# louissmit/VBNN

Hardware: AMD Instinct MI355X
Metric: VBLinear fwd+bwd samples/sec (higher is better)
Workload: dtype bf16; 1 GPU; 784-4096-4096-10 VBLinear MLP, batch 4096 per GPU, LRT, S=1; mode=lrt, global_batch=4096, parallelism=dp1, warmup_steps_run=255, backward_order=every updateGradInput, then the accGradParameters from the first layer up, launch=one stream launch per kernel

## Files before the change

include/vbnn_hip.h:

```cpp
#ifndef VBNN_HIP_H
#define VBNN_HIP_H

#include <stddef.h>
#include <stdint.h>

#ifdef __cplusplus
extern "C" {
#endif
#if defined(__GNUC__)
#pragma GCC visibility push(default)
#endif

#define VBNN_ABI_VERSION 6
#define VBNN_KPAD 64

enum { VBNN_OK = 0, VBNN_ERR_INVALID = 1, VBNN_ERR_HIP = 2, VBNN_ERR_NOMEM = 3, VBNN_ERR_UNSUPPORTED = 4 };
enum { VBNN_F32 = 0, VBNN_BF16 = 1 };
enum { VBNN_PACK_COPY = 0, VBNN_PACK_EXP = 1, VBNN_PACK_SQUARE = 2, VBNN_PACK_MUL = 3,
       VBNN_PACK_RELU = 4, VBNN_PACK_RELU_SQUARE = 5 };

typedef struct vbnn_ctx vbnn_ctx;

int vbnn_abi_version(void);
const char* vbnn_last_error(void);

#define VBNN_DEBUG_GEMM_KERNEL 0
#define VBNN_DEBUG_V2_SCHEDULE 1
#define VBNN_DEBUG_V2_TILE 2
#define VBNN_DEBUG_V3_MIN_K 4
#define VBNN_DEBUG_V2_PSPLIT 5
#define VBNN_DEBUG_V3_SPLIT 8
#define VBNN_DEBUG_V0 9
#define VBNN_DEBUG_HEAD_BACKWARD 10
#define VBNN_DEBUG_KMAJOR 6
int vbnn_debug_set(int key, int value);
#define VBNN_DEBUG_LAST_HEAD_FORM 11
#define VBNN_HEAD_ENTRY_FORWARD 1
#define VBNN_HEAD_ENTRY_SLOTS 2
#define VBNN_HEAD_ENTRY_STEP 3
#define VBNN_HEAD_ENTRY_TILE 4
#define VBNN_HEAD_ENTRY_STREAM 5
#define VBNN_HEAD_FINISH_NONE 0
#define VBNN_HEAD_FINISH_INLINE 1
#define VBNN_HEAD_FINISH_KERNEL 2
#define VBNN_HEAD_FORM(entry, bf16, vec, full, cp, finish) ((entry) | ((bf16) << 4) | ((vec) << 5) | ((full) << 6) | ((cp) << 8) | ((finish) << 16))
int vbnn_debug_get(int key);

int vbnn_kmajor_supported(int64_t M, int64_t N, int64_t K);
int vbnn_kmajor_supported_dw(int64_t I, int64_t O, int64_t N, int bias_row);
int vbnn_ctx_kmajor_supported(vbnn_ctx* ctx, int64_t M, int64_t N, int64_t K);
int vbnn_ctx_kmajor_supported_dw(vbnn_ctx* ctx, int64_t I, int64_t O, int64_t N, int bias_row);

int vbnn_ctx_create(int device, void* hip_stream, vbnn_ctx** out);
int vbnn_ctx_create_cu_budget(int device, int n_cus, vbnn_ctx** out);
int vbnn_ctx_stream(vbnn_ctx* ctx, void** hip_stream_out, int* n_cus_out);
int vbnn_ctx_destroy(vbnn_ctx* ctx);
int vbnn_ctx_set_stream(vbnn_ctx* ctx, void* hip_stream);
int vbnn_sync(vbnn_ctx* ctx);

int vbnn_buf_alloc(vbnn_ctx* ctx, size_t bytes, void** dptr);
int vbnn_buf_free(vbnn_ctx* ctx, void* dptr);
int vbnn_buf_zero(vbnn_ctx* ctx, void* dptr, size_t bytes);
int vbnn_buf_upload(vbnn_ctx* ctx, void* dst_dev, const void* src_host, size_t bytes);
int vbnn_buf_download(vbnn_ctx* ctx, void* dst_host, const void* src_dev, size_t bytes);

int vbnn_fill_normal(vbnn_ctx* ctx, float* out, int64_t rows, int64_t cols, int64_t ld,
                     uint64_t seed, uint32_t stream, uint32_t layer, uint32_t draw, int64_t row0,
                     float scale);
int vbnn_fill_normal_hw(vbnn_ctx* ctx, float* out, int64_t rows, int64_t cols, int64_t ld,
                        uint64_t seed, uint32_t stream, uint32_t layer, uint32_t draw, int64_t row0,
                        float scale);

int vbnn_box_muller_forms(vbnn_ctx* ctx, const uint32_t* x0, const uint32_t* x1, float* z_exact, float* z_hw, int64_t n);

int vbnn_compute_prior(vbnn_ctx* ctx, const float* means, const float* lvars, int64_t W,
                       float* vars, float* stdv, float* mu_sqe, double* stats);

int vbnn_wn_sample(vbnn_ctx* ctx, const float* means, const float* stdv, const float* lvars,
                   float* weight, float* e_out, int64_t O, int64_t I,
                   uint64_t seed, uint32_t layer, uint32_t draw);

int vbnn_pack(vbnn_ctx* ctx, int dtype, int func, const float* src, const float* src2, int64_t ld_src,
              int64_t rows, int64_t cols, void* dst, int64_t ld_dst, void* dstT, int64_t ld_dstT);


typedef struct vbnn_fwd_args {
    const void* w;
    const void* w2;
    const void* x;
    const void* x2;
    int64_t ld_w, ld_x;
    int64_t N, I, O;
    const float* bias;
    uint64_t seed; uint32_t layer; uint32_t draw; int64_t row0;
    float* y;  int64_t ld_y;
    void* r;  int64_t ld_r;
    int r_packed;
    int relu;
    void* h;  void* h2;  int64_t ld_h;
    void* hT; void* h2T; int64_t ld_hT;
    int64_t rows_per_draw;
    const uint32_t* draw_dev;
    const void* head_w3; int64_t head_ld_w; int64_t head_C; float* head_slots;
} vbnn_fwd_args;

int vbnn_forward(vbnn_ctx* ctx, int dtype, const vbnn_fwd_args* a);
int vbnn_forward_head_slots(vbnn_ctx* ctx, int dtype, int64_t N, int64_t I, int64_t O, int64_t C);

typedef struct vbnn_dx_args {
    const void* wT;
    const void* w2T;
    const void* g;
    const void* gv;
    int64_t ld_wT, ld_g;
    int64_t N, I, O;
    const void* x; int64_t ld_x;
    float* gx; int64_t ld_gx;
// ... 380 lines not shown
```

vbnn_amd/csrc/epilogues.h:

```cpp
#pragma once
#include "common.h"

template <typename T> struct V4;
template <> struct V4<float> { typedef f32x4 type; };
template <> struct V4<bf16_t> { typedef bf16x4 type; };
template <typename T>
__device__ __forceinline__ void store4_out(T* base, unsigned off, float a, float b, float c, float d) {
    vbnn_store_out(base, off, typename V4<T>::type{Elt<T>::to(a), Elt<T>::to(b), Elt<T>::to(c), Elt<T>::to(d)});
}

template <typename T>
struct EpiFwd {
    typedef T elem_t;
    const float* bias;
    int noise;
    uint64_t seed; uint32_t layer, draw; int64_t row0;
    const uint32_t* draw_dev = nullptr;
    int rpd;
    float* y; int64_t ld_y; int y_vec;
    float* r; T* r_t; int64_t ld_r; int r_vec;
    int relu;
    T* h; T* h2; int64_t ld_h;
    T* hT; T* h2T; int64_t ld_hT;
    int O, N;
// ... 64 lines not shown
            }
            if (STORE_T && hT) {
#pragma unroll
                for (int j = 0; j < 4; ++j)
                    if (j < valid) {
                        hT[(int64_t)(m + j) * ld_hT + n] = Elt<T>::to(t1[j]);
                        if (h2T) h2T[(int64_t)(m + j) * ld_hT + n] = Elt<T>::to(t2[j]);
                    }
            }
        }
    }
    __device__ __forceinline__ void operator()(int m, int n, f32x4 a1, f32x4 a2) const {
        float t1[4], t2[4];
        apply<true>(m, n, a1, a2, t1, t2);
    }

    static constexpr int FAST_BATCH = 8;
    static constexpr int FAST_BATCH_V2 = 4;
    struct Pre { f32x4 b; };
    struct Lane { int nl, ml; unsigned oh, orr; };
    __host__ __device__ __forceinline__ bool fast_ok() const {
        return !y && !r && h && (ld_h % 4 == 0) && (!r_t || (r_vec && ld_r % 8 == 0 && (((uintptr_t)r_t & 15u) == 0))) &&
               (!bias || (((uintptr_t)bias & 15u) == 0)) && (int64_t)N * ld_h < (1ll << 31) && (int64_t)N * ld_r < (1ll << 31);
    }
    __device__ __forceinline__ Lane lane_init(int nl, int ml) const {
        return Lane{nl, ml, (unsigned)(nl * (int)ld_h + ml), (unsigned)(nl * (int)ld_r + ml)};
    }
    __device__ __forceinline__ Pre load_fast(int um, int un, const Lane& ln) const {
        (void)un;
        Pre p;
        p.b = bias ? *reinterpret_cast<const f32x4*>(bias + um + ln.ml) : f32x4{0.f, 0.f, 0.f, 0.f};
        return p;
    }
    struct Noise { vbnn_f32x4 z; };
    __device__ __forceinline__ Noise draw_fast(int um, int un, const Lane& ln) const {
        Noise q = {};
        if (noise) q.z = zeta4(un + ln.nl, (uint32_t)((um + ln.ml) >> 2));
        return q;
    }
    __device__ __forceinline__ void apply_fast(int um, int un, const Lane& ln, f32x4 a1, f32x4 a2, const Pre& pre, float (&t1)[4],
                                               float (&t2)[4]) const {
        apply_fast_z(um, un, ln, a1, a2, pre, draw_fast(um, un, ln), t1, t2);
    }
    __device__ __forceinline__ void apply_fast_z(int um, int un, const Lane& ln, f32x4 a1, f32x4 a2, const Pre& pre, const Noise& q,
                                                 float (&t1)[4], float (&t2)[4]) const {
        float yv[4], rv[4];
        const vbnn_f32x4 z = q.z;
#pragma unroll
        for (int j = 0; j < 4; ++j) {
            const float mb = a1[j] + pre.b[j];
            if (noise) {
                const bool pos = a2[j] > 0.f;
                const float rs = __builtin_amdgcn_rsqf(a2[j]);
                const float sd = pos ? a2[j] * rs : 0.f;
                yv[j] = fmaf(sd, z.v[j], mb);
                rv[j] = pos ? 0.5f * z.v[j] * rs : 0.f;
            } else {
                yv[j] = mb;
                rv[j] = 0.f;
            }
        }
        if (r_t) store4_out<T>(r_t + ((int64_t)un * ld_r + um), ln.orr, rv[0], rv[1], rv[2], rv[3]);
#pragma unroll
        for (int j = 0; j < 4; ++j) {
            t1[j] = relu ? fmaxf(yv[j], 0.f) : yv[j];
            const float hr = Elt<T>::from(Elt<T>::to(t1[j]));
            t2[j] = hr * hr;
        }
        const int64_t ub = (int64_t)un * ld_h + um;
        store4_out<T>(h + ub, ln.oh, t1[0], t1[1], t1[2], t1[3]);
        if (h2) store4_out<T>(h2 + ub, ln.oh, t2[0], t2[1], t2[2], t2[3]);
    }

    static constexpr int FOLD_BATCH = 1;
    static constexpr int FOLD_SERIAL = 1;
    static constexpr int FOLD_STAGE = 1;
    typedef T fold_st_t;
    __host__ __device__ __forceinline__ T* fold_st_ptr() const { return r_t; }
    __host__ __device__ __forceinline__ int64_t fold_st_ld() const { return ld_r; }
    __host__ __device__ __forceinline__ const float* fold_bias_ptr() const { return bias; }
    __device__ __forceinline__ bool fold_st_stream() const { return h2 != nullptr; }
    __device__ __forceinline__ f32x4 fold_s(int um, int un, const Lane& ln, f32x4 v, const f32x4& b4, float (&rv)[4]) const {
        const vbnn_f32x4 z = normal4(seed, layer, draw, (uint32_t)(row0 + un + ln.nl), (uint32_t)((um + ln.ml) >> 2));
        f32x4 out;
#pragma unroll
        for (int j = 0; j < 4; ++j) {
            const bool pos = v[j] > 0.f;
            const float rs = __builtin_amdgcn_rsqf(v[j]);
            const float sd = pos ? v[j] * rs : 0.f;
            out[j] = fmaf(sd, z.v[j], b4[j]);
            rv[j] = pos ? 0.5f * z.v[j] * rs : 0.f;
        }
        return out;
    }
    struct FPre { f32x4 b; };
    __device__ __forceinline__ FPre fold_load(int um, int un, const Lane& ln) const {
        (void)un;
        FPre p;
        p.b = bias ? *reinterpret_cast<const f32x4*>(bias + um + ln.ml) : f32x4{0.f, 0.f, 0.f, 0.f};
        return p;
    }
    __device__ __forceinline__ f32x4 fold(int um, int un, const Lane& ln, f32x4 v, const FPre& fp) const {
        const vbnn_f32x4 z = normal4(seed, layer, draw, (uint32_t)(row0 + un + ln.nl), (uint32_t)((um + ln.ml) >> 2));
        f32x4 out;
        float rv[4];
#pragma unroll
        for (int j = 0; j < 4; ++j) {
            const bool pos = v[j] > 0.f;
            const float rs = __builtin_amdgcn_rsqf(v[j]);
            const float sd = pos ? v[j] * rs : 0.f;
            out[j] = fmaf(sd, z.v[j], fp.b[j]);
            rv[j] = pos ? 0.5f * z.v[j] * rs : 0.f;
        }
        if (r_t) store4_out<T>(r_t + ((int64_t)un * ld_r + um), ln.orr, rv[0], rv[1], rv[2], rv[3]);
        return out;
    }
    __device__ __forceinline__ bool folded_pre_needed() const { return false; }
    __device__ __forceinline__ Pre load_folded(int, int, const Lane&) const { return Pre{f32x4{0.f, 0.f, 0.f, 0.f}}; }
    __device__ __forceinline__ void apply_folded(int um, int un, const Lane& ln, f32x4 a, f32x4, const Pre&, float (&t1)[4],
                                                 float (&t2)[4]) const {
#pragma unroll
        for (int j = 0; j < 4; ++j) {
            t1[j] = relu ? fmaxf(a[j], 0.f) : a[j];
            const float hr = Elt<T>::from(Elt<T>::to(t1[j]));
            t2[j] = hr * hr;
        }
        const int64_t ub = (int64_t)un * ld_h + um;
        store4_out<T>(h + ub, ln.oh, t1[0], t1[1], t1[2], t1[3]);
        if (h2) store4_out<T>(h2 + ub, ln.oh, t2[0], t2[1], t2[2], t2[3]);
    }
};

template <typename T>
struct EpiDx {
    typedef T elem_t;
    int dual;
    const T* x; int64_t ld_x;
    float* gx; int64_t ld_gx; int gx_vec;
    int relu_mask;
    const float* r_prev; const T* r_prev_t; int64_t ld_r_prev; int r_vec;
    T* g_prev; T* gv_prev; int64_t ld_gp;
    T* gT_prev; T* gvT_prev; int64_t ld_gpT;
    int I, N;

    static constexpr bool SPLITTABLE = false;
    static constexpr bool EDGE_FAST = false;
    static constexpr bool HEAD = false;
    __device__ __forceinline__ void bind_draw() {}
    __host__ __device__ __forceinline__ bool has_draw_dev() const { return false; }
    __device__ __forceinline__ void edge_row(int, float) const {}
    __device__ __forceinline__ void set_part(int) {}
    __host__ __device__ __forceinline__ T* t1_ptr() const { return gT_prev; }
    __host__ __device__ __forceinline__ T* t2_ptr() const { return gvT_prev; }
    __host__ __device__ __forceinline__ int64_t t_ld() const { return ld_gpT; }
    __device__ __forceinline__ int m_dim() const { return I; }
    __device__ __forceinline__ int n_dim() const { return N; }
    __host__ __device__ __forceinline__ bool v3_ok() const { return true; }

    template <bool STORE_T>
    __device__ __forceinline__ void apply(int m, int n, f32x4 a1, f32x4 a2, float (&t1)[4], float (&t2)[4]) const {
        const int valid = min(4, I - m);
#pragma unroll
        for (int j = 0; j < 4; ++j) { t1[j] = 0.f; t2[j] = 0.f; }
        if (valid <= 0 || n >= N) return;
        float xv[4] = {0.f, 0.f, 0.f, 0.f};
        if (x) load4<T>(x + (int64_t)n * ld_x + m, xv, valid, (ld_x & 3) == 0);
// ... 316 lines not shown
```

vbnn_amd/csrc/gemm.hip:

```cpp
#include "gemm_dispatch.h"

extern "C" int vbnn_debug_set(int key, int value) {
    if (key == VBNN_DEBUG_GEMM_KERNEL && value >= 0 && value <= 3) { g_force_kernel = value; return VBNN_OK; }
    if (key == VBNN_DEBUG_V2_SCHEDULE && (value == -1 || value == 0 || value == 2 || value == 4)) { g_v2_sched = value; return VBNN_OK; }
    if (key == VBNN_DEBUG_V2_TILE && (value == 0 || value == 64 || value == 128 || value == 256)) { g_v2_tile = value; return VBNN_OK; }
    if (key == VBNN_DEBUG_V3_MIN_K && value >= 64) { g_v3_min_k = value; return VBNN_OK; }
    if (key == VBNN_DEBUG_V2_PSPLIT && value >= -1 && value <= 1) { g_v2_psplit = value; return VBNN_OK; }
    if (key == VBNN_DEBUG_KMAJOR && value >= 0 && value <= 2) { g_kmajor = value; return VBNN_OK; }
    if (key == VBNN_DEBUG_V3_SPLIT && value >= -1 && value <= 1) { g_v3_split = value; return VBNN_OK; }
    if (key == VBNN_DEBUG_V0 && (value == 0 || value == 1)) { g_v0 = value; return VBNN_OK; }
    if (key == VBNN_DEBUG_HEAD_BACKWARD && value >= -1 && value <= 1) { g_head_stream = value; return VBNN_OK; }
    vbnn_set_error("vbnn_debug_set: unknown key %d / value %d", key, value);
    return VBNN_ERR_INVALID;
}
extern "C" int vbnn_debug_get(int key) { return key == VBNN_DEBUG_LAST_HEAD_FORM ? g_last_head_form : -1; }

extern "C" int vbnn_kmajor_supported(int64_t M, int64_t N, int64_t K) { return kmajor_selected(M, N, K) ? 1 : 0; }
extern "C" int vbnn_ctx_kmajor_supported(vbnn_ctx* ctx, int64_t M, int64_t N, int64_t K) {
    vbnn_cu_scope plan(ctx);
    return kmajor_selected(M, N, K) ? 1 : 0;
}
extern "C" int vbnn_kmajor_supported_dw(int64_t I, int64_t O, int64_t N, int bias_row) {
    if (!bias_row && kmajor_selected(I, O, N)) return 1;
    if (I % 4 == 0 && kmajor_dw_v3_split_selected(I + (bias_row ? 1 : 0), O, N)) return 2;
    return kmajor_dw_v2_selected(I + (bias_row ? 1 : 0), O, N) ? 1 : 0;
}
extern "C" int vbnn_ctx_kmajor_supported_dw(vbnn_ctx* ctx, int64_t I, int64_t O, int64_t N, int bias_row) {
    vbnn_cu_scope plan(ctx);
    return vbnn_kmajor_supported_dw(I, O, N, bias_row);
}

extern "C" int vbnn_backward_pair(vbnn_ctx* ctx, int dtype, const vbnn_dx_args* dx, const vbnn_dw_args* dw) {
    VBNN_API_BEGIN
    vbnn_cu_scope plan(ctx);
    int chk = check_dx_args(ctx, dx);
    if (chk != VBNN_OK) return chk;
    chk = check_dw_args(ctx, dtype, dw);
    if (chk != VBNN_OK) return chk;
    VBNN_REQUIRE(dx->N == dw->N && dx->I == dw->I && dx->O == dw->O, "the two argument blocks describe one layer");
    if (dtype == VBNN_F32 && !dx->wT && dx->w && !dw->xT && dw->x && dw->g && dw->part == 0 && g_force_kernel == 0) {
        const bool dual = dx->gv != nullptr;
        const bool dw_dual = dw->gv != nullptr;
        if (dual == dw_dual && (!dual || (dx->w2 && !dw->x2))) {
            const EpiDx<float> ea = make_dx_epi<float>(dx);
            const EpiDw eb = make_dw_epi<float>(dw);
            const int M2 = (int)dw->I + (dw->gradBias ? 1 : 0);
            int st;
            if (dual)
                st = launch_gemm_v1_pair<true>(ctx->stream, (const float*)dx->w, (const float*)dx->w2, dx->ld_w, (const float*)dx->g,
                                               (const float*)dx->gv, dx->ld_g, (int)dx->I, (int)dx->N, (int)dx->O, ea, (const float*)dw->x,
                                               dw->ld_x, (const float*)dw->g, (const float*)dw->gv, dw->ld_g, M2, (int)dw->O, (int)dw->N,
                                               dw->gradBias ? (int)dw->I : -1, eb);
            else
                st = launch_gemm_v1_pair<false>(ctx->stream, (const float*)dx->w, nullptr, dx->ld_w, (const float*)dx->g, nullptr, dx->ld_g,
                                                (int)dx->I, (int)dx->N, (int)dx->O, ea, (const float*)dw->x, dw->ld_x, (const float*)dw->g,
                                                nullptr, dw->ld_g, M2, (int)dw->O, (int)dw->N, dw->gradBias ? (int)dw->I : -1, eb);
            if (st != VBNN_ERR_UNSUPPORTED) return st;
        }
    }
    int st = vbnn_acc_grad_parameters(ctx, dtype, dw);
    if (st != VBNN_OK) return st;
    return vbnn_grad_input(ctx, dtype, dx);
    VBNN_API_END
}
```

vbnn_amd/csrc/gemm_v3.h:

```cpp
#pragma once
#include "gemm_v2.h"

constexpr int V3_BM = 256, V3_BN = 256;
constexpr int V3_APART = 128 * 128;
constexpr int V3_BTILE = 256 * 128;
constexpr int V3_LDS = 4 * V3_APART + 3 * V3_BTILE;

inline int g_v3_min_k = 704;

#ifndef V3_ST
#define V3_ST(k) do { } while (0)
#endif


template <bool DUAL, bool AK, bool BK, class Epi, bool SPLIT = false, bool HM = false>
__global__ __launch_bounds__(512, 2) void gemm_nt_v3(const bf16_t* __restrict__ A, const bf16_t* __restrict__ A2, int64_t lda,
                                                     const bf16_t* __restrict__ B, const bf16_t* __restrict__ B2, int64_t ldb,
                                                     int M, int N, int nk, int tiles_m, int tiles_n, Epi epi_in) {
    static_assert(!(SPLIT && DUAL), "the split form computes one GEMM of the pair per workgroup");
    static_assert(SPLIT == HM && (!HM || (AK && BK)), "the pair-split launch is the half-height K-major form");
    extern __shared__ __attribute__((aligned(16))) unsigned char lds[];
    V3_ST(0);
    const int tid = threadIdx.x;
    const int lane = tid & 63;
    const int wave = __builtin_amdgcn_readfirstlane(tid >> 6);
    if (wave >= 4) __builtin_amdgcn_s_setprio(1);
    const int wr = wave >> 2, wc = wave & 3;
    Epi epi = epi_in;

    const int nblk = tiles_m * tiles_n * (SPLIT ? 2 : 1);
    int bid = blockIdx.x;
    {
        const int q = nblk >> 3, r = nblk & 7, xcd = bid & 7, idx = bid >> 3;
        bid = (xcd < r ? xcd * (q + 1) : r * (q + 1) + (xcd - r) * q) + idx;
    }
    if (SPLIT) {
        const int ntile = tiles_m * tiles_n;
        const int part = bid / ntile;
        bid -= part * ntile;
        epi.set_part(1 + part);
        if (part) { A = A2; B = B2; }
    }
    int tm, tn;
    {
        constexpr int GM = HM ? 8 : 4, GN = HM ? 4 : 8;
        const int per_band = GM * tiles_n;
        const int band = bid / per_band;
        const int in_band = bid - band * per_band;
        const int band_rows = min(GM, tiles_m - band * GM);
        const int full = band_rows * GN;
        const int grp = in_band / full;
        const int in_grp = in_band - grp * full;
        const int grp_cols = min(GN, tiles_n - grp * GN);
        tm = min(band * GM + in_grp / grp_cols, tiles_m - 1);
        tn = grp * GN + in_grp % grp_cols;
    }
    const int m0 = tm * (HM ? V3_BM / 2 : V3_BM), n0 = tn * V3_BN;

    int a_off[2][2], b_off[4];
    auto hk = [](int kr) { return (kr & 3) | (((kr >> 3) & 1) << 2); };
#pragma unroll
    for (int P = 0; P < 2; ++P)
#pragma unroll
        for (int d = 0; d < 2; ++d) {
            if (AK) {
                const int kr = 4 * (wave + 8 * d) + (lane >> 4);
                const int cs = (lane & 15) ^ (hk(kr) << 1);
                a_off[P][d] = kr * (int)lda + m0 + (cs >> 3) * (HM ? 64 : 128) + 64 * P + (cs & 7) * 8;
            } else {
                const int s = 8 * (wave + 8 * d) + (lane >> 3);
                const int row = (s >> 6) * 128 + 64 * P + (s & 63);
                const int chunk = (lane & 7) ^ ((s >> 1) & 7);
                a_off[P][d] = min(m0 + row, M - 1) * (int)lda + chunk * 8;
            }
        }
#pragma unroll
    for (int d = 0; d < 4; ++d) {
        if (BK) {
            const int kr = 2 * (wave + 8 * d) + (lane >> 5);
            const int cs = (lane & 31) ^ (hk(kr) << 1);
            b_off[d] = kr * (int)ldb + n0 + cs * 8;
        } else {
            const int row = 8 * (wave + 8 * d) + (lane >> 3);
            const int chunk = (lane & 7) ^ ((row >> 1) & 7);
            b_off[d] = min(n0 + row, N - 1) * (int)ldb + chunk * 8;
        }
    }
    const int a_kstep = AK ? V2_BK * (int)lda : V2_BK, b_kstep = BK ? V2_BK * (int)ldb : V2_BK;
    const bf16_t* Ap = A;
    const bf16_t* Bp = B;
#define V3_KT(t) (t)
#if defined(__HIP_DEVICE_COMPILE__)
    __amdgpu_buffer_rsrc_t ra = __builtin_amdgcn_make_buffer_rsrc((void*)Ap, 0, 0x7fffffff, 0x00020000);
    __amdgpu_buffer_rsrc_t rb = __builtin_amdgcn_make_buffer_rsrc((void*)Bp, 0, 0x7fffffff, 0x00020000);
#define V3_SET_OPERANDS(a_, b_) do { Ap = (a_); Bp = (b_); ra = __builtin_amdgcn_make_buffer_rsrc((void*)Ap, 0, 0x7fffffff, 0x00020000); \
                                     rb = __builtin_amdgcn_make_buffer_rsrc((void*)Bp, 0, 0x7fffffff, 0x00020000); } while (0)
#else
#define V3_SET_OPERANDS(a_, b_) do { Ap = (a_); Bp = (b_); } while (0)
// ... 324 lines not shown
        zero_acc();
        prologue();
        run_pass();
        V3_ST(5);
        v2_lds_barrier();
        if constexpr (Epi::FOLD_STAGE == 1) {
            constexpr int PITCH0 = 64 * (int)sizeof(typename Epi::fold_st_t) + 16, WSTG0 = 16 * PITCH0 + 512;
            const unsigned stg0 = (unsigned)(uintptr_t)(ldsb_t)(wave < 7 ? lds + 4 * V3_APART + 2 * V3_BTILE + wave * WSTG0
                                                                        : lds + 3 * V3_APART);
            int sl = lane;
            asm volatile("" : "+v"(sl));
            const float* bp = epi.fold_bias_ptr();
            f32x4 bq = f32x4{0.f, 0.f, 0.f, 0.f};
            if (bp) bq = *reinterpret_cast<const f32x4*>(bp + (m0 + wr * 128) + 4 * (sl & 31));
            asm volatile("ds_write_b128 %0, %1 offset:%2" ::"v"(stg0 + 16 * (sl & 31)), "v"(bq), "n"(16 * PITCH0) : "memory");
        }
        V3_SET_OPERANDS(A, B);
        prologue();
        int fc16 = c16, fq4 = q4, fm0 = m0 + wr * 128, fn0 = n0 + wc * 64;
        asm volatile("" : "+v"(fc16), "+v"(fq4), "+s"(fm0), "+s"(fn0));
        const typename Epi::Lane fln = epi.lane_init(fc16, 4 * fq4);
        auto fold_batch = [&](auto i0_c) {
            constexpr int i0 = decltype(i0_c)::value;
            constexpr int NB = Epi::FOLD_BATCH;
            typename Epi::FPre fp[NB][4];
#pragma unroll
            for (int b = 0; b < NB; ++b)
#pragma unroll
                for (int j = 0; j < 4; ++j) fp[b][j] = epi.fold_load(fm0 + 16 * (i0 + b), fn0 + 16 * j, fln);
#pragma unroll
            for (int b = 0; b < NB; ++b)
#pragma unroll
                for (int j = 0; j < 4; ++j) {
                    acc[i0 + b][j] = epi.fold(fm0 + 16 * (i0 + b), fn0 + 16 * j, fln, acc[i0 + b][j], fp[b][j]);
                    if (Epi::FOLD_SERIAL > 0 && (j % (Epi::FOLD_SERIAL > 0 ? Epi::FOLD_SERIAL : 1)) == Epi::FOLD_SERIAL - 1)
                        asm volatile("" : "+s"(fn0), "+s"(fm0)
                                     : "v"(acc[i0 + b][j][0]), "v"(acc[i0 + b][j][1]), "v"(acc[i0 + b][j][2]), "v"(acc[i0 + b][j][3]),
                                       "v"(acc[i0 + b][j ? j - 1 : 0][0]));
                }
        };
        static_assert(8 % Epi::FOLD_BATCH == 0, "FOLD_BATCH divides the 8 m-blocks of a wave tile");
        if constexpr (Epi::FOLD_STAGE == 2) {
            constexpr int PITCH = 64 * 4 + 16, WSTG = 16 * PITCH;
            static_assert(7 * WSTG <= V3_BTILE && WSTG <= V3_APART, "staging tiles must fit the free LDS");
            const unsigned stg = (unsigned)(uintptr_t)(ldsb_t)(wave < 7 ? lds + 4 * V3_APART + 2 * V3_BTILE + wave * WSTG
                                                                       : lds + 3 * V3_APART);
            int flane = lane;
            asm volatile("" : "+v"(flane));
            const unsigned wr_a = stg + fc16 * PITCH + 16 * fq4;
            const unsigned rd_a = stg + (flane >> 4) * PITCH + (flane & 15) * 16;
            float* const outp = epi.fold_st_ptr();
            const int64_t old = epi.fold_st_ld();
            const unsigned olane = (unsigned)((flane >> 4) * (int)old + (flane & 15) * 4);
            typename Epi::FPre fp[8][4];
#pragma unroll
            for (int b = 0; b < 8; ++b)
#pragma unroll
                for (int j = 0; j < 4; ++j) fp[b][j] = epi.fold_load(fm0 + 16 * b, fn0 + 16 * j, fln);
            const typename Epi::FoldK fk = epi.fold_k();
            auto fold_group = [&](auto g_c) {
                constexpr int G = decltype(g_c)::value;
#pragma unroll
                for (int j = 0; j < 4; ++j) {
#pragma unroll
                    for (int b = 0; b < 4; ++b) {
                        f32x4 sv;
                        acc[4 * G + b][j] = epi.fold_s(fk, acc[4 * G + b][j], fp[4 * G + b][j], sv);
                        asm volatile("ds_write_b128 %0, %1 offset:%2" ::"v"(wr_a), "v"(sv), "n"(64 * b) : "memory");
                    }
                    f32x4 r0, r1, r2, r3;
                    asm volatile("ds_read_b128 %0, %4\n\tds_read_b128 %1, %4 offset:%5\n\tds_read_b128 %2, %4 offset:%6\n\t"
                                 "ds_read_b128 %3, %4 offset:%7\n\ts_waitcnt lgkmcnt(0)"
                                 : "=&v"(r0), "=&v"(r1), "=&v"(r2), "=&v"(r3)
                                 : "v"(rd_a), "n"(4 * PITCH), "n"(8 * PITCH), "n"(12 * PITCH) : "memory");
                    float* const row0p = outp + ((int64_t)(fn0 + 16 * j) * old + fm0 + 64 * G);
                    vbnn_store_grad(row0p, olane, r0);
                    vbnn_store_grad(row0p + 4 * old, olane, r1);
                    vbnn_store_grad(row0p + 8 * old, olane, r2);
                    vbnn_store_grad(row0p + 12 * old, olane, r3);
                }
            };
            fold_group(std::integral_constant<int, 0>());
            fold_group(std::integral_constant<int, 1>());
        } else if constexpr (Epi::FOLD_STAGE != 0) {
            typedef typename Epi::fold_st_t ST;
            static_assert(sizeof(ST) == 2, "staging tile geometry: 64 m x 2 bytes = one 128-byte row segment");
            constexpr int PITCH = 64 * (int)sizeof(ST) + 16;
            constexpr int WSTG = 16 * PITCH + 512;
            static_assert(7 * WSTG <= V3_BTILE && WSTG <= V3_APART, "staging tiles must fit the free LDS");
            const unsigned stg = (unsigned)(uintptr_t)(ldsb_t)(wave < 7 ? lds + 4 * V3_APART + 2 * V3_BTILE + wave * WSTG
                                                                       : lds + 3 * V3_APART);
            const unsigned wr_a = stg + fc16 * PITCH + 8 * fq4;
            int flane = lane;
            asm volatile("" : "+v"(flane));
            const unsigned bias_a = stg + 16 * fq4;
            const unsigned rd_a = stg + (flane >> 3) * PITCH + (flane & 7) * 16;
            ST* const outp = epi.fold_st_ptr();
            const int64_t old = epi.fold_st_ld();
            const bool st_stream = epi.fold_st_stream();
            const unsigned olane = (unsigned)((flane >> 3) * (int)old + (flane & 7) * 8);
            auto fold_group = [&](auto g_c) {
                constexpr int G = decltype(g_c)::value;
#pragma unroll
                for (int j = 0; j < 4; ++j) {
#pragma unroll
                    for (int b = 0; b < 4; ++b) {
                        f32x4 b4;
                        asm volatile("ds_read_b128 %0, %1 offset:%2\n\ts_waitcnt lgkmcnt(0)" : "=&v"(b4) : "v"(bias_a), "n"(16 * PITCH + 64 * (4 * G + b)) : "memory");
                        float sv[4];
                        acc[4 * G + b][j] = epi.fold_s(fm0 + 16 * (4 * G + b), fn0 + 16 * j, fln, acc[4 * G + b][j], b4, sv);
                        const bf16x4 pk = bf16x4{Elt<ST>::to(sv[0]), Elt<ST>::to(sv[1]), Elt<ST>::to(sv[2]), Elt<ST>::to(sv[3])};
                        asm volatile("ds_write_b64 %0, %1 offset:%2" ::"v"(wr_a), "v"(pk), "n"(32 * b) : "memory");
                        if (Epi::FOLD_SERIAL > 0)
                            asm volatile("" : "+s"(fn0), "+s"(fm0)
                                         : "v"(acc[4 * G + b][j][0]), "v"(acc[4 * G + b][j][1]), "v"(acc[4 * G + b][j][2]), "v"(acc[4 * G + b][j][3]));
                    }
                    bf16x8 r0, r1;
                    asm volatile("ds_read_b128 %0, %2\n\tds_read_b128 %1, %2 offset:%3\n\ts_waitcnt lgkmcnt(0)"
                                 : "=&v"(r0), "=&v"(r1) : "v"(rd_a), "n"(8 * PITCH) : "memory");
                    ST* const row0p = outp + ((int64_t)(fn0 + 16 * j) * old + fm0 + 64 * G);
                    vbnn_store_stream(row0p, olane, r0, st_stream);
                    vbnn_store_stream(row0p + 8 * old, olane, r1, st_stream);
                }
            };
            fold_group(std::integral_constant<int, 0>());
            fold_group(std::integral_constant<int, 1>());
        } else {
        fold_batch(std::integral_constant<int, 0>());
        if constexpr (Epi::FOLD_BATCH < 8) fold_batch(std::integral_constant<int, Epi::FOLD_BATCH>());
        if constexpr (Epi::FOLD_BATCH < 4) {
            fold_batch(std::integral_constant<int, 2 * Epi::FOLD_BATCH>()); fold_batch(std::integral_constant<int, 3 * Epi::FOLD_BATCH>());
        }
        if constexpr (Epi::FOLD_BATCH < 2) {
            fold_batch(std::integral_constant<int, 4>()); fold_batch(std::integral_constant<int, 5>());
            fold_batch(std::integral_constant<int, 6>()); fold_batch(std::integral_constant<int, 7>());
        }
        }
        V3_ST(6);
        run_pass();
    } else {
        zero_acc();
        if constexpr (HM) prologue_hm_pp(); else prologue();
        run_pass();
    }
    __syncthreads();
    V3_ST(1);

    if constexpr (!SPLIT && Epi::HEAD) {
        if (epi.head_slots) {
            const int hq4 = lane >> 4, hc16 = lane & 15;
            const bf16_t* wrow = epi.head_w3 + (int64_t)min(hc16, epi.head_C - 1) * epi.head_ld_w + (m0 + wr * 128) + 4 * hq4;
            bf16x8 wf[4];
#pragma unroll
            for (int pr = 0; pr < 4; ++pr) {
                const bf16x4 lo = *reinterpret_cast<const bf16x4*>(wrow + 32 * pr);
                const bf16x4 hi = *reinterpret_cast<const bf16x4*>(wrow + 32 * pr + 16);
                wf[pr] = __builtin_shufflevector(lo, hi, 0, 1, 2, 3, 4, 5, 6, 7);
            }
            const bool relu = epi.relu != 0;
            float* const sl = epi.head_slots + ((int64_t)(tm * 2 + wr) * epi.N + (n0 + wc * 64)) * 16 + hc16 * 16 + 4 * hq4;
            f32x4 hbias[8];
#pragma unroll
            for (int i = 0; i < 8; ++i) hbias[i] = f32x4{0.f, 0.f, 0.f, 0.f};
            if constexpr (!DUAL) {
                const float* bp = epi.fold_bias_ptr();
                if (bp) {
// ... 80 lines not shown
#pragma unroll
            for (int b = 0; b < FB; ++b) {
                const int p = p0 + b;
                float t1[4], t2[4];
                if (DUAL) epi.apply_folded(wm0, wn0 + 4 * p, eln, r1[p], r2[p], pre[b], t1, t2);
                else epi.apply_fast(wm0, wn0 + 4 * p, eln, r1[p], f32x4{0.f, 0.f, 0.f, 0.f}, pre[b], t1, t2);
                if (any_t) {
                    const int nl = 4 * p + q4;
                    const int col = ((nl >> 3) ^ (c16 & 3)) * 8 + (nl & 7);
#pragma unroll
                    for (int j = 0; j < 4; ++j) {
                        tl1[(4 * c16 + j) * TQ + col] = Elt<ET>::to(t1[j]);
                        tl2[(4 * c16 + j) * TQ + col] = Elt<ET>::to(t2[j]);
                    }
                }
                __builtin_amdgcn_sched_barrier(0);
            }
        }
        if (any_t) {
            const int64_t ldt = epi.t_ld();
            const unsigned lo = (unsigned)((lane >> 2) * (int)ldt + 8 * (lane & 3));
#pragma unroll
            for (int pp = 0; pp < 4; ++pp) {
                const int ml = 16 * pp + (lane >> 2);
                const int64_t ub = (int64_t)(wm0 + 16 * pp) * ldt + wn0;
                if (tp1)
                    *reinterpret_cast<bf16x8*>(tp1 + ub + lo) =
                        *reinterpret_cast<const bf16x8*>(tl1 + ml * TQ + 8 * ((lane & 3) ^ ((ml >> 2) & 3)));
                if (tp2)
                    *reinterpret_cast<bf16x8*>(tp2 + ub + lo) =
                        *reinterpret_cast<const bf16x8*>(tl2 + ml * TQ + 8 * ((lane & 3) ^ ((ml >> 2) & 3)));
            }
        }
    });
    V3_ST(4);
}

template <class Epi>
static inline bool gemm_v3_possible(int64_t M, int64_t N, int64_t K, int64_t lda, int64_t ldb, bool ak, bool bk, const Epi& epi) {
    Epi e = epi;
    const bool t_ok = (!e.t1_ptr() && !e.t2_ptr()) ||
                      ((e.t_ld() % 8 == 0) && ((((uintptr_t)e.t1_ptr() | (uintptr_t)e.t2_ptr()) & 15u) == 0));
    const bool a_ok = ak ? (K % V2_BK == 0 && lda % 8 == 0 && lda >= M && K * lda < (1ll << 30)) : M * lda < (1ll << 30);
    const bool b_ok = bk ? (K % V2_BK == 0 && ldb % 8 == 0 && ldb >= N && K * ldb < (1ll << 30)) : N * ldb < (1ll << 30);
    return (M % V3_BM == 0) && (N % V3_BN == 0) && a_ok && b_ok && epi.fast_ok() && epi.v3_ok() && t_ok && M * e.t_ld() < (1ll << 31);
}
static inline bool gemm_v3_shape_ok(int64_t M, int64_t N, int64_t K) {
    if (M % V3_BM || N % V3_BN || K < g_v3_min_k) return false;
    const int64_t cus = vbnn_cu_count();
    const int64_t t3 = (M / V3_BM) * (N / V3_BN), t2 = 2 * t3;
    if (4 * t3 < 3 * cus) return false;
    const int64_t r3 = (t3 + cus - 1) / cus, r2 = (t2 + cus - 1) / cus;
    return 185 * r3 <= 100 * r2;
}
template <class Epi>
static inline bool gemm_v3_eligible(int64_t M, int64_t N, int64_t K, int64_t lda, int64_t ldb, bool ak, bool bk, const Epi& epi) {
    if (!gemm_v3_possible(M, N, K, lda, ldb, ak, bk, epi) || K < g_v3_min_k) return false;
    const int64_t cus = vbnn_cu_count();
    const int64_t t3 = (M / V3_BM) * (N / V3_BN), t2 = 2 * t3;
    if (4 * t3 < 3 * cus) return false;
    const int64_t r3 = (t3 + cus - 1) / cus, r2 = (t2 + cus - 1) / cus;
    return 185 * r3 <= 100 * r2;
}

template <typename T, bool DUAL, bool AK, bool BK, class Epi>
static int launch_gemm_v3(vbnn_ctx* ctx, const T* A, const T* A2, int64_t lda, const T* B, const T* B2, int64_t ldb, int M, int N,
                          int K, const Epi& epi) {
    if constexpr (sizeof(T) != 2) {
        vbnn_set_error("gemm_v3 is bf16 only");
        return VBNN_ERR_UNSUPPORTED;
    } else {
        if ((((uintptr_t)A | (uintptr_t)B | (uintptr_t)A2 | (uintptr_t)B2) & 15u) != 0) {
            vbnn_set_error("gemm_v3 operands must be 16-byte aligned");
            return VBNN_ERR_INVALID;
        }
        const int nk = (K + V2_BK - 1) / V2_BK;
        if ((!AK && lda < (int64_t)nk * V2_BK) || (!BK && ldb < (int64_t)nk * V2_BK)) {
            vbnn_set_error("packed leading dimension too small for K=%d", K);
            return VBNN_ERR_INVALID;
        }
        if (!gemm_v3_possible(M, N, K, lda, ldb, AK, BK, epi)) { vbnn_set_error("gemm_v3: shape / outputs outside its fast path"); return VBNN_ERR_UNSUPPORTED; }
        const int tiles_m = (M + V3_BM - 1) / V3_BM, tiles_n = (N + V3_BN - 1) / V3_BN;
        const void* kern = (const void*)gemm_nt_v3<DUAL, AK, BK, Epi>;
        static vbnn_per_device_flag configured_on;
        bool& configured = configured_on[ctx->device];
        if (!configured) {
            hipError_t e = hipFuncSetAttribute(kern, hipFuncAttributeMaxDynamicSharedMemorySize, V3_LDS);
            if (e != hipSuccess) { vbnn_set_error("hipFuncSetAttribute: %s", hipGetErrorString(e)); return VBNN_ERR_HIP; }
            configured = true;
        }
        const bf16_t* a = (const bf16_t*)A; const bf16_t* a2 = (const bf16_t*)A2;
        const bf16_t* b = (const bf16_t*)B; const bf16_t* b2 = (const bf16_t*)B2;
        int nk_ = nk, M_ = M, N_ = N, tm_ = tiles_m, tn_ = tiles_n;
        int64_t lda_ = lda, ldb_ = ldb;
        Epi epi_ = epi;
        void* args[] = {&a, &a2, &lda_, &b, &b2, &ldb_, &M_, &N_, &nk_, &tm_, &tn_, &epi_};
        hipError_t e = hipLaunchKernel(kern, dim3(tiles_m * tiles_n), dim3(512), args, V3_LDS, ctx->stream);
        if (e != hipSuccess) { vbnn_set_error("launch of gemm_nt_v3 failed: %s", hipGetErrorString(e)); return VBNN_ERR_HIP; }
        return vbnn_check_launch("gemm_nt_v3");
    }
}

inline int g_v3_split = -1;
static inline bool gemm_v3_split_shape_ok(int64_t M, int64_t N, int64_t K) {
    if (g_v3_split == 0 || N % V3_BN || K % V2_BK) return false;
    if (g_v3_split == 1) return true;
    const int64_t tiles = ((M + V3_BM - 1) / V3_BM) * (N / V3_BN);
    const int64_t blocks = ((M + V3_BM / 2 - 1) / (V3_BM / 2)) * (N / V3_BN) * 2;
    const int64_t cus = vbnn_cu_count();
    return tiles * 16 <= 5 * cus && tiles * 16 >= 3 * cus && K >= 2048 && blocks <= cus && blocks * 8 >= 5 * cus;
}
static inline int64_t gemm_v3_split_lda(int64_t M) { return (M + V3_BM - 1) / V3_BM * V3_BM; }

template <typename T, class Epi>
static int launch_gemm_v3_split(vbnn_ctx* ctx, const T* A, const T* A2, int64_t lda, const T* B, const T* B2, int64_t ldb, int M, int N,
                                int K, const Epi& epi) {
    if constexpr (sizeof(T) != 2 || !Epi::SPLITTABLE || !Epi::EDGE_FAST) {
        return VBNN_ERR_UNSUPPORTED;
    } else {
        Epi e0 = epi;
        if (!A || !A2 || !B || !B2 || !gemm_v3_split_shape_ok(M, N, K) || !epi.fast_ok() || e0.t1_ptr() || e0.t2_ptr() ||
            (((uintptr_t)A | (uintptr_t)B | (uintptr_t)A2 | (uintptr_t)B2) & 15u) != 0 || lda % 8 || ldb % 8 ||
            lda < gemm_v3_split_lda(M) || ldb < N || (int64_t)K * lda >= (1ll << 30) || (int64_t)K * ldb >= (1ll << 30))
            return VBNN_ERR_UNSUPPORTED;
        const int tiles_n = N / V3_BN;
        const int tiles_m = (M + V3_BM / 2 - 1) / (V3_BM / 2);
        const void* kern = (const void*)gemm_nt_v3<false, true, true, Epi, true, true>;
        static vbnn_per_device_flag configured_on;
        bool& configured = configured_on[ctx->device];
        if (!configured) {
            hipError_t e = hipFuncSetAttribute(kern, hipFuncAttributeMaxDynamicSharedMemorySize, V3_LDS);
            if (e != hipSuccess) { vbnn_set_error("hipFuncSetAttribute: %s", hipGetErrorString(e)); return VBNN_ERR_HIP; }
            configured = true;
        }
        const bf16_t* a = (const bf16_t*)A; const bf16_t* a2 = (const bf16_t*)A2;
        const bf16_t* b = (const bf16_t*)B; const bf16_t* b2 = (const bf16_t*)B2;
        int nk_ = K / V2_BK, M_ = M, N_ = N, tm_ = tiles_m, tn_ = tiles_n;
        int64_t lda_ = lda, ldb_ = ldb;
        Epi epi_ = epi;
        void* args[] = {&a, &a2, &lda_, &b, &b2, &ldb_, &M_, &N_, &nk_, &tm_, &tn_, &epi_};
        hipError_t e = hipLaunchKernel(kern, dim3(tiles_m * tiles_n * 2), dim3(512), args, V3_LDS, ctx->stream);
        if (e != hipSuccess) { vbnn_set_error("launch of gemm_nt_v3 (pair split) failed: %s", hipGetErrorString(e)); return VBNN_ERR_HIP; }
        return vbnn_check_launch("gemm_nt_v3 pair split");
    }
}
```

Before: 5.439 million samples/s.

## Software-pipeline Philox noise generation with staged stores in v3 forward fold epilogue

Adds a pipelined variant of the gemm_v3 fold epilogue for the forward LRT epilogue. It computes the next group's Philox words while the current group's staged LDS rows are read back and stored, and it prefetches the bias. The serial path stays behind a new debug key. The aim is to hide RNG ALU latency and LDS/global store latency in the epilogue, at the cost of more registers and hand-written waitcnt ordering.

Result: faster. 5.541 million samples/s, median of 6 (+1.9%).

```diff
diff --git a/include/vbnn_hip.h b/include/vbnn_hip.h
--- a/include/vbnn_hip.h
+++ b/include/vbnn_hip.h
@@ -33,6 +33,7 @@
 #define VBNN_DEBUG_V0 9
 #define VBNN_DEBUG_HEAD_BACKWARD 10
 #define VBNN_DEBUG_KMAJOR 6
+#define VBNN_DEBUG_V3_FOLD_SERIAL 12
 int vbnn_debug_set(int key, int value);
 #define VBNN_DEBUG_LAST_HEAD_FORM 11
 #define VBNN_HEAD_ENTRY_FORWARD 1
diff --git a/vbnn_amd/csrc/epilogues.h b/vbnn_amd/csrc/epilogues.h
--- a/vbnn_amd/csrc/epilogues.h
+++ b/vbnn_amd/csrc/epilogues.h
@@ -170,6 +170,36 @@
     __device__ __forceinline__ bool fold_st_stream() const { return h2 != nullptr; }
     __device__ __forceinline__ f32x4 fold_s(int um, int un, const Lane& ln, f32x4 v, const f32x4& b4, float (&rv)[4]) const {
         const vbnn_f32x4 z = normal4(seed, layer, draw, (uint32_t)(row0 + un + ln.nl), (uint32_t)((um + ln.ml) >> 2));
+        f32x4 out;
+#pragma unroll
+        for (int j = 0; j < 4; ++j) {
+            const bool pos = v[j] > 0.f;
+            const float rs = __builtin_amdgcn_rsqf(v[j]);
+            const float sd = pos ? v[j] * rs : 0.f;
+            out[j] = fmaf(sd, z.v[j], b4[j]);
+            rv[j] = pos ? 0.5f * z.v[j] * rs : 0.f;
+        }
+        return out;
+    }
+    static constexpr int FOLD_PIPE = 1;
+    __device__ __forceinline__ vbnn_u32x4 fold_words(int um, int un, const Lane& ln) const {
+        return vbnn_philox4x32_10((uint32_t)((um + ln.ml) >> 2), (uint32_t)(row0 + un + ln.nl), draw, (layer << 8) | VBNN_STREAM_ZETA,
+                                  (uint32_t)seed, (uint32_t)(seed >> 32));
+    }
+    static __device__ __forceinline__ vbnn_f32x4 fold_z(const vbnn_u32x4& u) {
+        vbnn_f32x4 z;
+#ifndef VBNN_BF16_EXACT_NORMALS
+        if constexpr (sizeof(T) == 2) {
+            vbnn_box_muller_hw(u.v[0], u.v[1], &z.v[0], &z.v[1]);
+            vbnn_box_muller_hw(u.v[2], u.v[3], &z.v[2], &z.v[3]);
+            return z;
+        }
+#endif
+        vbnn_box_muller(u.v[0], u.v[1], &z.v[0], &z.v[1]);
+        vbnn_box_muller(u.v[2], u.v[3], &z.v[2], &z.v[3]);
+        return z;
+    }
+    static __device__ __forceinline__ f32x4 fold_sz(f32x4 v, const f32x4& b4, const vbnn_f32x4& z, float (&rv)[4]) {
         f32x4 out;
 #pragma unroll
         for (int j = 0; j < 4; ++j) {
diff --git a/vbnn_amd/csrc/gemm.hip b/vbnn_amd/csrc/gemm.hip
--- a/vbnn_amd/csrc/gemm.hip
+++ b/vbnn_amd/csrc/gemm.hip
@@ -10,6 +10,7 @@
     if (key == VBNN_DEBUG_V3_SPLIT && value >= -1 && value <= 1) { g_v3_split = value; return VBNN_OK; }
     if (key == VBNN_DEBUG_V0 && (value == 0 || value == 1)) { g_v0 = value; return VBNN_OK; }
     if (key == VBNN_DEBUG_HEAD_BACKWARD && value >= -1 && value <= 1) { g_head_stream = value; return VBNN_OK; }
+    if (key == VBNN_DEBUG_V3_FOLD_SERIAL && (value == 0 || value == 1)) { g_v3_fold_serial = value; return VBNN_OK; }
     vbnn_set_error("vbnn_debug_set: unknown key %d / value %d", key, value);
     return VBNN_ERR_INVALID;
 }
diff --git a/vbnn_amd/csrc/gemm_v3.h b/vbnn_amd/csrc/gemm_v3.h
--- a/vbnn_amd/csrc/gemm_v3.h
+++ b/vbnn_amd/csrc/gemm_v3.h
@@ -7,13 +7,16 @@
 constexpr int V3_LDS = 4 * V3_APART + 3 * V3_BTILE;
 
 inline int g_v3_min_k = 704;
+inline int g_v3_fold_serial = 0;
+template <class Epi, class = void> struct v3_fold_pipe { static constexpr int value = 0; };
+template <class Epi> struct v3_fold_pipe<Epi, std::void_t<decltype(Epi::FOLD_PIPE)>> { static constexpr int value = Epi::FOLD_PIPE; };
 
 #ifndef V3_ST
 #define V3_ST(k) do { } while (0)
 #endif
 
 
-template <bool DUAL, bool AK, bool BK, class Epi, bool SPLIT = false, bool HM = false>
+template <bool DUAL, bool AK, bool BK, class Epi, bool SPLIT = false, bool HM = false, int PIPE = v3_fold_pipe<Epi>::value>
 __global__ __launch_bounds__(512, 2) void gemm_nt_v3(const bf16_t* __restrict__ A, const bf16_t* __restrict__ A2, int64_t lda,
                                                      const bf16_t* __restrict__ B, const bf16_t* __restrict__ B2, int64_t ldb,
                                                      int M, int N, int nk, int tiles_m, int tiles_n, Epi epi_in) {
@@ -504,6 +507,92 @@
             };
             fold_group(std::integral_constant<int, 0>());
             fold_group(std::integral_constant<int, 1>());
+        } else if constexpr (Epi::FOLD_STAGE != 0 && PIPE != 0) {
+            typedef typename Epi::fold_st_t ST;
+            typedef uint32_t u32x4 __attribute__((ext_vector_type(4)));
+            static_assert(sizeof(ST) == 2, "staging tile geometry: 64 m x 2 bytes = one 128-byte row segment");
+            constexpr int PITCH = 64 * (int)sizeof(ST) + 16;
+            constexpr int WSTG = 16 * PITCH + 512;
+            static_assert(7 * WSTG <= V3_BTILE && WSTG <= V3_APART, "staging tiles must fit the free LDS");
+            const unsigned stg = (unsigned)(uintptr_t)(ldsb_t)(wave < 7 ? lds + 4 * V3_APART + 2 * V3_BTILE + wave * WSTG
+                                                                       : lds + 3 * V3_APART);
+            const unsigned wr_a = stg + fc16 * PITCH + 8 * fq4;
+            int flane = lane;
+            asm volatile("" : "+v"(flane));
+            const unsigned bias_a = stg + 16 * fq4;
+            const unsigned rd_a = stg + (flane >> 3) * PITCH + (flane & 7) * 16;
+            ST* const outp = epi.fold_st_ptr();
+            const int64_t old = epi.fold_st_ld();
+            const bool st_stream = epi.fold_st_stream();
+            const unsigned olane = (unsigned)((flane >> 3) * (int)old + (flane & 7) * 8);
+            auto words = [&](auto g_c, u32x4 (&u)[4]) {
+                constexpr int G = decltype(g_c)::value >> 2, j = decltype(g_c)::value & 3;
+#pragma unroll
+                for (int b = 0; b < 4; ++b) {
+                    const vbnn_u32x4 w = epi.fold_words(fm0 + 16 * (4 * G + b), fn0 + 16 * j, fln);
+                    u[b] = u32x4{w.v[0], w.v[1], w.v[2], w.v[3]};
+                }
+            };
+            auto store_rows = [&](auto g_c, const bf16x8& r0, const bf16x8& r1) {
+                constexpr int G = decltype(g_c)::value >> 2, j = decltype(g_c)::value & 3;
+                ST* const row0p = outp + ((int64_t)(fn0 + 16 * j) * old + fm0 + 64 * G);
+                vbnn_store_stream(row0p, olane, r0, st_stream);
+                vbnn_store_stream(row0p + 8 * old, olane, r1, st_stream);
+            };
+            u32x4 uw[4];
+            f32x4 b4[4];
+#define V3_FOLD_READ_BIAS(G)                                                                                                        \
+    asm volatile("ds_read_b128 %0, %5 offset:%6\n\tds_read_b128 %1, %5 offset:%7\n\tds_read_b128 %2, %5 offset:%8\n\t"                    \
+                 "ds_read_b128 %3, %5 offset:%9"                                                                                     \
+                 : "=&v"(b4[0]), "=&v"(b4[1]), "=&v"(b4[2]), "=&v"(b4[3]), "+s"(fn0)                                                 \
+                 : "v"(bias_a), "n"(16 * PITCH + 256 * (G)), "n"(16 * PITCH + 256 * (G) + 64), "n"(16 * PITCH + 256 * (G) + 128),    \
+                   "n"(16 * PITCH + 256 * (G) + 192) : "memory")
+            V3_FOLD_READ_BIAS(0);
+            words(std::integral_constant<int, 0>(), uw);
+            asm volatile("s_waitcnt lgkmcnt(0)" : "+v"(b4[0]), "+v"(b4[1]), "+v"(b4[2]), "+v"(b4[3]),
+                         "+v"(uw[0]), "+v"(uw[1]), "+v"(uw[2]), "+v"(uw[3]), "+s"(fn0), "+s"(fm0) :: "memory");
+            vbnn_static_for<0, 8>([&](auto g_c) {
+                constexpr int g = decltype(g_c)::value, G = g >> 2, j = g & 3;
+                [[maybe_unused]] bf16x8 r0, r1;
+                [[maybe_unused]] u32x4 un[4];
+                if constexpr (g > 0)
+                    asm volatile("ds_read_b128 %0, %3\n\tds_read_b128 %1, %3 offset:%4"
+                                 : "=&v"(r0), "=&v"(r1), "+s"(fn0) : "v"(rd_a), "n"(8 * PITCH) : "memory");
+#pragma unroll
+                for (int b = 0; b < 4; ++b) {
+                    const vbnn_f32x4 z = Epi::fold_z(vbnn_u32x4{{uw[b][0], uw[b][1], uw[b][2], uw[b][3]}});
+                    float sv[4];
+                    acc[4 * G + b][j] = Epi::fold_sz(acc[4 * G + b][j], b4[b], z, sv);
+                    const bf16x4 pk = bf16x4{Elt<ST>::to(sv[0]), Elt<ST>::to(sv[1]), Elt<ST>::to(sv[2]), Elt<ST>::to(sv[3])};
+                    asm volatile("ds_write_b64 %0, %1 offset:%2" ::"v"(wr_a), "v"(pk), "n"(32 * b) : "memory");
+                }
+                asm volatile("" : "+s"(fn0), "+s"(fm0)
+                             : "v"(acc[4 * G][j]), "v"(acc[4 * G + 1][j]), "v"(acc[4 * G + 2][j]), "v"(acc[4 * G + 3][j]));
+                if constexpr (g == 3) V3_FOLD_READ_BIAS(1);
+                if constexpr (g < 7) words(std::integral_constant<int, g + 1>(), un);
+                if constexpr (g == 0)
+                    asm volatile("" : "+v"(un[0]), "+v"(un[1]), "+v"(un[2]), "+v"(un[3]), "+s"(fn0), "+s"(fm0));
+                else if constexpr (g == 3)
+                    asm volatile("s_waitcnt lgkmcnt(0)" : "+v"(r0), "+v"(r1), "+v"(b4[0]), "+v"(b4[1]), "+v"(b4[2]), "+v"(b4[3]),
+                                 "+v"(un[0]), "+v"(un[1]), "+v"(un[2]), "+v"(un[3]), "+s"(fn0), "+s"(fm0) :: "memory");
+                else if constexpr (g < 7)
+                    asm volatile("s_waitcnt lgkmcnt(0)" : "+v"(r0), "+v"(r1), "+v"(un[0]), "+v"(un[1]), "+v"(un[2]), "+v"(un[3]),
+                                 "+s"(fn0), "+s"(fm0) :: "memory");
+                else
+                    asm volatile("s_waitcnt lgkmcnt(0)" : "+v"(r0), "+v"(r1), "+s"(fn0), "+s"(fm0) :: "memory");
+                if constexpr (g > 0) store_rows(std::integral_constant<int, g - 1>(), r0, r1);
+                if constexpr (g < 7) {
+#pragma unroll
+                    for (int b = 0; b < 4; ++b) uw[b] = un[b];
+                }
+            });
+            {
+                bf16x8 r0, r1;
+                asm volatile("ds_read_b128 %0, %2\n\tds_read_b128 %1, %2 offset:%3\n\ts_waitcnt lgkmcnt(0)"
+                             : "=&v"(r0), "=&v"(r1) : "v"(rd_a), "n"(8 * PITCH) : "memory");
+                store_rows(std::integral_constant<int, 7>(), r0, r1);
+            }
+#undef V3_FOLD_READ_BIAS
         } else if constexpr (Epi::FOLD_STAGE != 0) {
             typedef typename Epi::fold_st_t ST;
             static_assert(sizeof(ST) == 2, "staging tile geometry: 64 m x 2 bytes = one 128-byte row segment");
@@ -750,8 +839,12 @@
         if (!gemm_v3_possible(M, N, K, lda, ldb, AK, BK, epi)) { vbnn_set_error("gemm_v3: shape / outputs outside its fast path"); return VBNN_ERR_UNSUPPORTED; }
         const int tiles_m = (M + V3_BM - 1) / V3_BM, tiles_n = (N + V3_BN - 1) / V3_BN;
         const void* kern = (const void*)gemm_nt_v3<DUAL, AK, BK, Epi>;
-        static vbnn_per_device_flag configured_on;
-        bool& configured = configured_on[ctx->device];
+        int form = 0;
+        if constexpr (DUAL && v3_fold_pipe<Epi>::value != 0) {
+            if (g_v3_fold_serial) { kern = (const void*)gemm_nt_v3<DUAL, AK, BK, Epi, false, false, 0>; form = 1; }
+        }
+        static vbnn_per_device_flag configured_on[2];
+        bool& configured = configured_on[form][ctx->device];
         if (!configured) {
             hipError_t e = hipFuncSetAttribute(kern, hipFuncAttributeMaxDynamicSharedMemorySize, V3_LDS);
             if (e != hipSuccess) { vbnn_set_error("hipFuncSetAttribute: %s", hipGetErrorString(e)); return VBNN_ERR_HIP; }
```
